# xuchang116/smCounter

Measured on NVIDIA B200. Metric: target_loci_called_per_sec, higher is better.
Workload: dtype int32+f64

## Files before the change

### smcounter_b200/csrc/smc_api.cu

```cuda
#include <chrono>
#include <cmath>
#include <cstdio>
#include <cstdlib>
#include <new>
#include <mutex>
#include <string>
#include <vector>

#include <nvtx3/nvToolsExt.h>

#include "smc_common.cuh"
#include "smc_sort.cuh"
#include "smc_pileup.cuh"
#include "smc_stats.cuh"

namespace {

struct NvtxRange {
    explicit NvtxRange(const char* name) { nvtxRangePushA(name); }
    ~NvtxRange() { nvtxRangePop(); }
};

thread_local std::string g_create_error;
static std::mutex g_link_mu;
// ... 341 lines not shown
        return SMC_E_CUDA;
    }
    if (device < 0 || device >= ndev) { g_create_error = "smc_ctx_create: bad device index"; return SMC_E_ARG; }
    smc_ctx* ctx = new (std::nothrow) smc_ctx();
    if (!ctx) { g_create_error = "smc_ctx_create: out of host memory"; return SMC_E_ARG; }
    ctx->device = device; ctx->prm = *params;
    if (const char* ev = getenv("SMC_CHUNK")) { long v = atol(ev); if (v >= 64 && v <= 1000000) ctx->chunk = (uint32_t)v; }
    auto fail = [&](const char* what, cudaError_t ce) {
        g_create_error = std::string(what) + ": " + cudaGetErrorString(ce);
        delete ctx; return SMC_E_CUDA;
    };
    if ((e = cudaSetDevice(device)) != cudaSuccess) return fail("cudaSetDevice", e);
    if ((e = cudaStreamCreateWithFlags(&ctx->st, cudaStreamNonBlocking)) != cudaSuccess) return fail("cudaStreamCreate", e);
    for (DevBuf* b : all_bufs(ctx)) b->st = ctx->st;
    {
        cudaMemPool_t pool;
        unsigned long long keep = ~0ull;
        if ((e = cudaDeviceGetDefaultMemPool(&pool, device)) != cudaSuccess) return fail("cudaDeviceGetDefaultMemPool", e);
        if ((e = cudaMemPoolSetAttribute(pool, cudaMemPoolAttrReleaseThreshold, &keep)) != cudaSuccess) return fail("cudaMemPoolSetAttribute", e);
    }
    for (auto& ev : ctx->ev) if ((e = cudaEventCreate(&ev)) != cudaSuccess) return fail("cudaEventCreate", e);
    if ((e = cudaStreamCreateWithFlags(&ctx->st_copy, cudaStreamNonBlocking)) != cudaSuccess) return fail("cudaStreamCreate", e);
    if ((e = cudaEventCreateWithFlags(&ctx->ev_scal, cudaEventDisableTiming)) != cudaSuccess) return fail("cudaEventCreate", e);
    if ((e = cudaEventCreateWithFlags(&ctx->ev_link, cudaEventDisableTiming)) != cudaSuccess) return fail("cudaEventCreate", e);
    if ((e = cudaEventCreateWithFlags(&ctx->ev_tmp, cudaEventDisableTiming)) != cudaSuccess) return fail("cudaEventCreate", e);
    if ((e = cudaEventCreateWithFlags(&ctx->ev_tmp2, cudaEventDisableTiming)) != cudaSuccess) return fail("cudaEventCreate", e);
    for (auto& ev : ctx->ev_chunk) if ((e = cudaEventCreateWithFlags(&ev, cudaEventDisableTiming)) != cudaSuccess) return fail("cudaEventCreate", e);
    std::vector<double> bq(256);
    for (int q = 0; q < 256; ++q) bq[q] = std::pow(10.0, -(double)q / 10.0);
    const size_t per = (size_t)(PCR_NMAX + 1) * (PCR_NMAX + 2) / 2;
    std::vector<double> pcr(3 * per);
    for (int k = 4; k <= 6; ++k)
        for (int n = 0; n <= PCR_NMAX; ++n)
            for (int c = 0; c <= n; ++c) {
                double ratio = ((double)c + 0.5) / ((double)n + 0.5 * (double)k);
                pcr[(size_t)(k - 4) * per + (size_t)n * (n + 1) / 2 + c] = std::pow(10.0, -6.0 * ratio);
            }
    if ((e = ctx->d_bqtab.ensure(256 * 8)) != cudaSuccess) return fail("cudaMalloc", e);
    if ((e = ctx->d_pcrtab.ensure(pcr.size() * 8)) != cudaSuccess) return fail("cudaMalloc", e);
    cudaMemcpy(ctx->d_bqtab.p, bq.data(), 256 * 8, cudaMemcpyHostToDevice);
    cudaMemcpy(ctx->d_pcrtab.p, pcr.data(), pcr.size() * 8, cudaMemcpyHostToDevice);
    if ((e = cudaFuncSetAttribute(k_merge_t<false>, cudaFuncAttributeMaxDynamicSharedMemorySize, KB_SMEM_BYTES)) != cudaSuccess)
        return fail("cudaFuncSetAttribute(k_merge)", e);
    if ((e = cudaFuncSetAttribute(k_merge_t<true>, cudaFuncAttributeMaxDynamicSharedMemorySize, KB_SMEM_BYTES)) != cudaSuccess)
        return fail("cudaFuncSetAttribute(k_merge list)", e);
    if ((e = cudaFuncSetAttribute(k_gather_t<false>, cudaFuncAttributeMaxDynamicSharedMemorySize, KA_SMEM_BYTES(false))) != cudaSuccess)
        return fail("cudaFuncSetAttribute(k_gather)", e);
    if ((e = cudaFuncSetAttribute(k_gather_t<true>, cudaFuncAttributeMaxDynamicSharedMemorySize, KA_SMEM_BYTES(true))) != cudaSuccess)
        return fail("cudaFuncSetAttribute(k_gather list)", e);
    cudaFuncSetAttribute(k_gather_t<false>, cudaFuncAttributePreferredSharedMemoryCarveout, cudaSharedmemCarveoutMaxShared);
    cudaFuncSetAttribute(k_gather_t<true>, cudaFuncAttributePreferredSharedMemoryCarveout, cudaSharedmemCarveoutMaxShared);
    cudaFuncSetAttribute(k_merge_t<false>, cudaFuncAttributePreferredSharedMemoryCarveout, cudaSharedmemCarveoutMaxShared);
    cudaFuncSetAttribute(k_merge_t<true>, cudaFuncAttributePreferredSharedMemoryCarveout, cudaSharedmemCarveoutMaxShared);
    if ((e = radix_sort_init()) != cudaSuccess) return fail("cudaFuncSetAttribute(k_radix_scatter)", e);
    if ((e = ctx->d_small.ensure(4096)) != cudaSuccess) return fail("cudaMalloc", e);
    *out = ctx;
    return SMC_OK;
}

extern "C" void smc_ctx_destroy(smc_ctx* ctx) {
    if (!ctx) return;
    cudaSetDevice(ctx->device);
    if (ctx->st_copy) cudaStreamSynchronize(ctx->st_copy);
    cudaStreamSynchronize(ctx->st);
    for (DevBuf* b : all_bufs(ctx)) b->release();
    cudaStreamSynchronize(ctx->st);
    for (auto& ev : ctx->ev) if (ev) cudaEventDestroy(ev);
    for (auto& ev : ctx->ev_chunk) if (ev) cudaEventDestroy(ev);
    if (ctx->ev_scal) cudaEventDestroy(ctx->ev_scal);
    if (ctx->ev_tmp) cudaEventDestroy(ctx->ev_tmp);
    if (ctx->ev_tmp2) cudaEventDestroy(ctx->ev_tmp2);
    if (ctx->ev_link) {
        std::lock_guard<std::mutex> lk(g_link_mu);
        if (ctx->device >= 0 && ctx->device < 64 && g_link_owner[ctx->device] == ctx) { g_link_owner[ctx->device] = nullptr; g_link_tail[ctx->device] = nullptr; }
        cudaEventDestroy(ctx->ev_link);
    }
    if (ctx->st_copy) cudaStreamDestroy(ctx->st_copy);
    if (ctx->st) cudaStreamDestroy(ctx->st);
    delete ctx;
}

static int pipe_chunks_for(const smc_reads_soa* R) {
    if (const char* ev = getenv("SMC_PIPE_CHUNKS")) { long v = atol(ev); if (v >= 1 && v <= SMC_PIPE_MAX) return (int)v; }
    const int64_t payload = R->seq_bytes + R->qual_bytes;
    if (R->n_reads < 65536 || payload < (96ll << 20)) return 1;
    const int64_t g = payload / (48ll << 20);
    return (int)(g < 2 ? 2 : g > 12 ? 12 : g);
}

static int upload_impl(smc_ctx* ctx, const smc_reads_soa* R, const smc_loci* Lc, const smc_umi_keep* K, bool pipelined) {
    if (!ctx) return SMC_E_ARG;
    NvtxRange nvtx_r("smc:upload");
    if (!R || !Lc) { ctx->err = "smc_upload: null reads/loci"; return SMC_E_ARG; }
    if (R->n_reads < 0 || Lc->n_loci < 0) { ctx->err = "smc_upload: negative size"; return SMC_E_ARG; }
    if (Lc->n_loci > SMC_MAX_LOCI) { ctx->err = "smc_upload: more than 4194302 loci in one batch"; return SMC_E_LIMIT; }
    if (R->n_reads > (1ll << 30) || R->seq_bytes >= (1ll << 32) || R->qual_bytes >= (1ll << 32) || R->n_cigar_words >= (1ll << 32)) {
        ctx->err = "smc_upload: batch exceeds 2^30 reads or 4 GiB of bases/qualities/cigar; split the batch"; return SMC_E_LIMIT;
    }
    CK(cudaSetDevice(ctx->device));
    ctx->uploaded = false; ctx->ran = false;
    const int64_t n = R->n_reads, nl = Lc->n_loci;
    const int G = pipelined ? pipe_chunks_for(R) : 1;
    ctx->pipe_n = 0;
    const bool split = pipelined && G > 1;
    cudaStream_t up_st = split ? ctx->st_copy : ctx->st;
    static const bool link_turns = [] { const char* ev = getenv("SMC_LINK_TURNS"); return !(ev && atoi(ev) == 0); }();
    std::unique_lock<std::mutex> link_lock(g_link_mu, std::defer_lock);
// ... 182 lines not shown
            LAUNCH(k_chunk_reads, 1, 32, 0, ctx->d_qual_poff.as<uint32_t>(), n, (uint32_t)R->qual_bytes, ctx->pipe_qual_chunk, G,
                   ctx->d_small.as<uint32_t>() + SW_CHUNK_READS);
        if (sbits == 2)
            LAUNCH(k_chunk_reads, 1, 32, 0, ctx->d_seq_poff.as<uint32_t>(), n, (uint32_t)R->seq_bytes, ctx->pipe_seq_chunk, G,
                   ctx->d_small.as<uint32_t>() + SW_CHUNK_READS_SEQ);
        grew = true;
        ALLOC_SYNC();
        for (int c = 0; c < G; ++c) {
            const int64_t s0 = std::min<int64_t>(R->seq_bytes, (int64_t)c * ctx->pipe_seq_chunk), s1 = std::min<int64_t>(R->seq_bytes, (int64_t)(c + 1) * ctx->pipe_seq_chunk);
            const int64_t q0 = std::min<int64_t>(R->qual_bytes, (int64_t)c * ctx->pipe_qual_chunk), q1 = std::min<int64_t>(R->qual_bytes, (int64_t)(c + 1) * ctx->pipe_qual_chunk);
            if (s1 > s0) CK(cudaMemcpyAsync(seq_up.as<uint8_t>() + s0, R->seq + s0, (size_t)(s1 - s0), cudaMemcpyHostToDevice, ctx->st_copy));
            if (q1 > q0) CK(cudaMemcpyAsync(qual_up.as<uint8_t>() + q0, R->qual + q0, (size_t)(q1 - q0), cudaMemcpyHostToDevice, ctx->st_copy));
            CK(cudaEventRecord(ctx->ev_chunk[c], ctx->st_copy));
            bytes += (s1 - s0) + (q1 - q0);
        }
        CK(cudaEventRecord(ctx->ev[1], ctx->st_copy));
        if (link_lock.owns_lock()) {
            CK(cudaEventRecord(ctx->ev_link, ctx->st_copy));
            g_link_tail[dv] = ctx->ev_link; g_link_owner[dv] = ctx;
        }
        ctx->pipe_n = G;
    }
#undef UP
#undef SYNC_UP
#undef ENSURE
#undef ALLOC_SYNC
    ctx->tm.pipe_chunks = pipelined ? G : 0;
    ctx->tm.bytes_h2d = bytes;
    ctx->uploaded = true;
    return SMC_OK;
}

extern "C" int smc_upload(smc_ctx* ctx, const smc_reads_soa* R, const smc_loci* Lc, const smc_umi_keep* K) {
    return upload_impl(ctx, R, Lc, K, false);
}

static int run_pileup_and_stats(smc_ctx* ctx, uint32_t n_tiles, int64_t NE);

extern "C" int smc_run_resident(smc_ctx* ctx) {
    if (!ctx) return SMC_E_ARG;
    if (!ctx->uploaded) { ctx->err = "smc_run_resident: nothing uploaded"; return SMC_E_STATE; }
    CK(cudaSetDevice(ctx->device));
    g_launches = 0;
    NvtxRange nvtx_r("smc:read_sort+prep+tile_events");
    const int64_t n = ctx->n_reads, nl = ctx->n_loci;
    const uint32_t n_tiles = (uint32_t)((nl + 31) / 32);
    uint32_t* small = ctx->d_small.as<uint32_t>();
    CK(cudaEventRecord(ctx->ev[2], ctx->st));
    int64_t NE = 0;
    int frag_bits_used = 32;
    if (n > 0 && nl > 0) {
        CK(ctx->d_k0.ensure((size_t)n * 8)); CK(ctx->d_k1.ensure((size_t)n * 8));
        CK(ctx->d_v0.ensure((size_t)n * 4)); CK(ctx->d_v1.ensure((size_t)n * 4));
        CK(ctx->d_hist.ensure(radix_hist_words(n) * 4 + 1024));
        CK(ctx->d_scan.ensure((size_t)std::max<int64_t>(radix_scan_words(n), scan_scratch_words(n + 1)) * 4 + 1024));
        uint64_t* k0 = ctx->d_k0.as<uint64_t>(); uint64_t* k1 = ctx->d_k1.as<uint64_t>();
        uint32_t* v0 = ctx->d_v0.as<uint32_t>(); uint32_t* v1 = ctx->d_v1.as<uint32_t>();
        int slot_bits = 4;
        while ((double)(1ll << slot_bits) < 1.1 * (double)n) ++slot_bits;
        int frag_bits = 1;
        while ((1ll << frag_bits) < n) ++frag_bits;
        frag_bits_used = frag_bits;
        CK(ctx->d_umi_table.ensure(((size_t)1 << slot_bits) * 8));
        CK(cudaMemsetAsync(ctx->d_umi_table.p, 0xff, ((size_t)1 << slot_bits) * 8, ctx->st));
        CK(cudaMemsetAsync(small + SW_FRAG_OR, 0, 8, ctx->st));
        LAUNCH(k_umi_slots, nblk(n, 256), 256, 0, ctx->d_umi.as<uint64_t>(), ctx->d_frag.as<uint32_t>(), n,
               ctx->d_umi_table.as<unsigned long long>(), (uint32_t)((1u << slot_bits) - 1u), frag_bits, k0, v0, (unsigned long long*)(small + SW_FRAG_OR));
        CK(cudaEventRecord(ctx->ev[11], ctx->st));
        if (radix_sort_bits(k0, v0, k1, v1, n, 0, slot_bits + frag_bits, ctx->d_hist.as<uint32_t>(), ctx->d_scan.as<uint32_t>(), ctx->st)) {
            std::swap(k0, k1); std::swap(v0, v1);
        }
        CK(cudaEventRecord(ctx->ev[12], ctx->st));
        ctx->tm.read_sort_passes = (slot_bits + frag_bits + RS_MAX_BITS - 1) / RS_MAX_BITS;
        const uint32_t* perm = v0;
        CK(ctx->d_urank.ensure((size_t)n * 4)); CK(ctx->d_frank.ensure((size_t)n * 4));
        CK(ctx->d_umi_of_urank.ensure((size_t)n * 8));
        uint32_t* uex = ctx->d_urank.as<uint32_t>(); uint32_t* fex = ctx->d_frank.as<uint32_t>();
        {
            const int64_t nbt = (n + SCAN_TILE - 1) / SCAN_TILE;
            uint32_t* scr = ctx->d_scan.as<uint32_t>();
            CK(cudaMemsetAsync(scr, 0, (size_t)(2 * nbt + 8) * 4, ctx->st));
            LAUNCH(k_rank_scan, (unsigned)nbt, SCAN_THREADS, 0, k0, frag_bits, n, ctx->d_umi.as<uint64_t>(), perm, uex, fex,
                   ctx->d_umi_of_urank.as<uint64_t>(), v1, reinterpret_cast<unsigned long long*>(scr + 2), scr, small + SW_N_UMI);
        }
        CK(ctx->d_recs.ensure((size_t)n * sizeof(ReadRec))); CK(ctx->d_grec.ensure((size_t)n * sizeof(GRec)));
        CK(cudaMemsetAsync(small + SW_N_TILE_EVENTS, 0, 32, ctx->st));
        PrepArgs P{};
        ctx->inv_ptr = v1;
        P.n_reads = n; P.inv = v1; P.urank = uex; P.frank = fex;
        P.ref_id = ctx->d_ref_id.as<int32_t>(); P.pos = ctx->d_pos.as<int32_t>(); P.flag = ctx->d_flag.as<uint16_t>();
        P.mapq = ctx->d_mapq.as<uint8_t>(); P.nm = ctx->d_nm.as<int32_t>(); P.l_seq = ctx->d_lseq.as<int32_t>();
        P.seq_off = ctx->d_seq_off.as<int64_t>(); P.qual_off = ctx->d_qual_off.as<int64_t>(); P.cigar_off = ctx->d_cig_off.as<int64_t>();
        P.n_cigar = ctx->d_ncig.as<uint16_t>(); P.cigar = ctx->d_cigar.as<uint32_t>();
        if (ctx->has_store) { P.store_lo = ctx->d_store_lo.as<int32_t>(); P.store_len = ctx->d_store_len.as<int32_t>(); }
        P.loci_key = ctx->d_loci_key.as<uint64_t>(); P.n_loci = nl;
        P.minMQ = ctx->prm.minMQ; P.primerDist = ctx->prm.primerDist; P.mismatchThr = ctx->prm.mismatchThr;
        P.recs = ctx->d_recs.as<ReadRec>(); P.grec = ctx->d_grec.as<GRec>(); P.gflags = small + SW_GFLAGS;
        if (ctx->pipe_n > 1) {
            CK(ctx->d_pipe_need.ensure((size_t)n));
            P.pipe_need = ctx->d_pipe_need.as<uint8_t>(); P.pipe_n = (uint32_t)ctx->pipe_n;
            P.pipe_seq_chunk = ctx->pipe_seq_chunk; P.pipe_qual_chunk = ctx->pipe_qual_chunk;
            if (ctx->qual_bits != 8) { P.qual_poff = ctx->d_qual_poff.as<uint32_t>(); P.qual_bits = ctx->qual_bits; }
            if (ctx->seq_bits == 2) P.seq_poff = ctx->d_seq_poff.as<uint32_t>();
        }
        CK(cudaEventRecord(ctx->ev[13], ctx->st));
        LAUNCH(k_read_prep, nblk(n, 256), 256, 0, P);
        CK(cudaEventRecord(ctx->ev[14], ctx->st));
        ctx->tm.read_prep_bytes = n * (int64_t)(4 + 4 + 2 + 1 + 4 + 4 + 8 + 8 + 8 + 2 + (ctx->has_store ? 8 : 0) + 4 + sizeof(ReadRec) + sizeof(GRec)) + 4 * ctx->n_cigar_words;
        if (ctx->ne_cap < 4 * n + 4096) ctx->ne_cap = 4 * n + 4096;
        for (int attempt = 0; attempt < 2; ++attempt) {
            if (ctx->ne_cap > 0xfffffff0ll) ctx->ne_cap = 0xfffffff0ll;
            CK(ctx->d_ek0.ensure((size_t)ctx->ne_cap * 8)); CK(ctx->d_ev0.ensure((size_t)ctx->ne_cap * 4));
            const int64_t nbt = (n + SCAN_TILE - 1) / SCAN_TILE;
            uint32_t* scr = ctx->d_scan.as<uint32_t>();
            CK(cudaMemsetAsync(scr, 0, (size_t)(2 * nbt + 8) * 4, ctx->st));
            LAUNCH(k_expand_scan, (unsigned)nbt, SCAN_THREADS, 0, ctx->d_recs.as<ReadRec>(), n, ctx->d_ek0.as<uint64_t>(), ctx->d_ev0.as<uint32_t>(),
                   (uint32_t)ctx->ne_cap, reinterpret_cast<unsigned long long*>(scr + 2), scr, small + SW_N_TILE_EVENTS);
            if (attempt == 1) break;
        uint32_t h[2], tot[5];
        unsigned long long frag_or = 0;
        CK(cudaMemcpyAsync(&frag_or, small + SW_FRAG_OR, 8, cudaMemcpyDeviceToHost, ctx->st));
        CK(cudaMemcpyAsync(h, small + SW_N_TILE_EVENTS, 8, cudaMemcpyDeviceToHost, ctx->st));
        CK(cudaMemcpyAsync(tot, small + SW_PACK_TOTALS, 20, cudaMemcpyDeviceToHost, ctx->st));
        CK(cudaStreamSynchronize(ctx->st));
        if (h[1] & GF_BAD_READ) { ctx->err = "a read has l_seq or clip length > 65535 (unsupported)"; return SMC_E_LIMIT; }
        if (h[1] & GF_BAD_STORE) {
            ctx->err = "stored window: store_lo must be even and >= 0, store_lo + store_len <= l_seq, reads with indels / clips inside must be "
                       "stored whole, and every target base of a read must lie inside its window";
            return SMC_E_ARG;
        }
        if (frag_or >> frag_bits_used) { ctx->err = "frag_id must be a dense id (< n_reads), numbered by first appearance"; return SMC_E_ARG; }
        if ((ctx->packed_seq && (int64_t)tot[ctx->seq_bits == 2 ? 4 : 0] != ctx->seq_bytes) || (ctx->packed_qual && (int64_t)tot[ctx->qual_bits != 8 ? 3 : 1] != ctx->qual_bytes) ||
            (ctx->packed_cigar && (int64_t)tot[2] != ctx->n_cigar_words)) {
            ctx->err = "packed payload (NULL offsets): seq_bytes / qual_bytes / n_cigar_words do not match the sums of (len+1)/2, len, n_cigar (len = store_len or l_seq)";
            return SMC_E_ARG;
        }
            NE = h[0];
            if (NE <= ctx->ne_cap) break;
            ctx->ne_cap = NE + NE / 8 + 4096;
        }
    }
    CK(cudaEventRecord(ctx->ev[3], ctx->st));
    CK(cudaEventRecord(ctx->ev[15], ctx->st));
    const uint64_t* ev_key_sorted = nullptr; const uint32_t* ev_read_sorted = nullptr;
    CK(ctx->d_tile_off.ensure((size_t)(n_tiles + 2) * 4)); CK(ctx->d_unit_cnt.ensure((size_t)(n_tiles + 2) * 4));
    CK(ctx->d_unit_off.ensure((size_t)(n_tiles + 2) * 4));
    if (NE > 0) {
        CK(ctx->d_ek1.ensure((size_t)NE * 8)); CK(ctx->d_ev1.ensure((size_t)NE * 4));
        CK(ctx->d_hist.ensure(radix_hist_words(NE) * 4 + 1024));
        CK(ctx->d_scan.ensure((size_t)std::max<int64_t>(radix_scan_words(NE), scan_scratch_words((int64_t)n_tiles + 2)) * 4 + 1024));
        int tile_bits = 0;
        while (((uint64_t)(n_tiles - 1) >> tile_bits) != 0) ++tile_bits;
        int res = radix_sort_bits(ctx->d_ek0.as<uint64_t>(), ctx->d_ev0.as<uint32_t>(), ctx->d_ek1.as<uint64_t>(), ctx->d_ev1.as<uint32_t>(),
                                  NE, 0, tile_bits, ctx->d_hist.as<uint32_t>(), ctx->d_scan.as<uint32_t>(), ctx->st);
        ev_key_sorted = res ? ctx->d_ek1.as<uint64_t>() : ctx->d_ek0.as<uint64_t>();
        ev_read_sorted = res ? ctx->d_ev1.as<uint32_t>() : ctx->d_ev0.as<uint32_t>();
    } else {
        CK(ctx->d_scan.ensure((size_t)scan_scratch_words((int64_t)n_tiles + 2) * 4 + 1024));
    }
    CK(cudaEventRecord(ctx->ev[16], ctx->st));
    LAUNCH(k_tile_offsets, nblk((int64_t)n_tiles + 1, 256), 256, 0, ev_key_sorted, NE, n_tiles, ctx->chunk, ctx->d_tile_off.as<uint32_t>(),
           ctx->d_unit_cnt.as<uint32_t>());
    exclusive_scan_u32(ctx->d_unit_cnt.as<uint32_t>(), ctx->d_unit_off.as<uint32_t>(), (int64_t)n_tiles + 1, ctx->d_scan.as<uint32_t>(),
                       nullptr, ctx->st);
    {
        const int64_t max_units = (int64_t)n_tiles + NE / ctx->chunk + 1;
        ctx->n_units_cap = (uint32_t)max_units;
        CK(ctx->d_unit_eb.ensure((size_t)max_units * 4)); CK(ctx->d_unit_ee.ensure((size_t)max_units * 4));
        CK(ctx->d_unit_tile.ensure((size_t)max_units * 4)); CK(ctx->d_unit_nfrag.ensure((size_t)max_units * 4));
        LAUNCH(k_unit_bounds, nblk(max_units, 256), 256, 0, ctx->d_tile_off.as<uint32_t>(), ctx->d_unit_off.as<uint32_t>(), n_tiles, ctx->chunk,
               ev_read_sorted, ctx->d_urank.as<uint32_t>(), ctx->d_unit_eb.as<uint32_t>(), ctx->d_unit_ee.as<uint32_t>(), ctx->d_unit_tile.as<uint32_t>(),
               ctx->n_units_cap);
    }
    ctx->tm.n_tile_events = NE;
    ctx->ev_read_sorted = ev_read_sorted;
    ctx->n_tiles = n_tiles; ctx->n_tile_events = NE;
    (void)ev_key_sorted;
    if (ctx->pipe_n > 1 && NE > 0) {
        const int G = ctx->pipe_n;
        uint32_t init[SMC_PIPE_MAX];
        for (int c = 0; c < SMC_PIPE_MAX; ++c) init[c] = ctx->n_units_cap;
        uint32_t* pd = small + SW_PIPE_BLOCKED;
        CK(cudaMemcpyAsync(pd, init, sizeof(init), cudaMemcpyHostToDevice, ctx->st));
        LAUNCH(k_pipe_unit_need, nblk((int64_t)ctx->n_units_cap * 32, 256), 256, 0, ctx->d_unit_eb.as<uint32_t>(),
               ctx->d_unit_ee.as<uint32_t>(), ev_read_sorted, ctx->d_pipe_need.as<uint8_t>(), ctx->n_units_cap, pd);
        uint32_t h[SMC_PIPE_MAX];
        CK(cudaMemcpyAsync(h, pd, sizeof(h), cudaMemcpyDeviceToHost, ctx->st));
        CK(cudaStreamSynchronize(ctx->st));
        uint32_t run = ctx->n_units_cap;
        for (int c = G - 1; c >= 0; --c) {
            if (c < G - 1) run = std::min(run, h[c]);
            ctx->pipe_end[c] = run;
        }
    }
    CK(cudaEventRecord(ctx->ev[4], ctx->st));
    return run_pileup_and_stats(ctx, n_tiles, NE);
}


static DynTab make_dyntab(smc_ctx* ctx) {
    uint32_t* small = ctx->d_small.as<uint32_t>();
    DynTab T;
    T.dkey = ctx->d_dkey.as<unsigned long long>(); T.dmask = ctx->dyn_cap - 1; T.drep_read = ctx->d_drep_read.as<uint32_t>();
    T.drep_qpos = ctx->d_drep_qpos.as<int32_t>(); T.dlen = ctx->d_dlen.as<int32_t>(); T.dcnt = ctx->d_dcnt.as<int32_t>();
    T.dlimb = ctx->d_dlimb.as<unsigned long long>(); T.diskey = ctx->d_diskey.as<uint8_t>(); T.dcount = small + SW_DYN_COUNT; T.gflags = small + SW_GFLAGS;
    T.seq = ctx->d_seq.as<uint8_t>(); T.seq_off = ctx->d_seq_off.as<int64_t>();
    T.spill = ctx->d_spill.as<SpillRec>(); T.spill_cap = ctx->spill_cap; T.spill_count = small + SW_SPILL_COUNT;
// ... 418 lines not shown
```

### smcounter_b200/csrc/smc_sort.cuh

```cuda
#pragma once
#include "smc_common.cuh"

#define SCAN_THREADS 256
#define SCAN_ITEMS   8
#define SCAN_TILE    (SCAN_THREADS * SCAN_ITEMS)

__global__ void __launch_bounds__(SCAN_THREADS)
k_scan_tile(const uint32_t* in, uint32_t* out, int64_t n, uint32_t* sums) {
    __shared__ uint32_t warp_tot[SCAN_THREADS / 32];
    int64_t base = (int64_t)blockIdx.x * SCAN_TILE + (int64_t)threadIdx.x * SCAN_ITEMS;
    uint32_t v[SCAN_ITEMS];
    uint32_t tsum = 0;
#pragma unroll
    for (int i = 0; i < SCAN_ITEMS; ++i) {
        v[i] = (base + i < n) ? in[base + i] : 0u;
        tsum += v[i];
    }
    uint32_t incl = tsum;
#pragma unroll
    for (int d = 1; d < 32; d <<= 1) {
        uint32_t t = __shfl_up_sync(FULL_MASK, incl, d);
        if (lane_id() >= (uint32_t)d) incl += t;
    }
    int w = threadIdx.x >> 5;
// ... 63 lines not shown
    for (int d = 1; d < 32; d <<= 1) {
        uint32_t t = __shfl_up_sync(FULL_MASK, incl, d);
        if (lane_id() >= (uint32_t)d) incl += t;
    }
    const int w = threadIdx.x >> 5;
    if (lane_id() == 31) warp_tot[w] = incl;
    __syncthreads();
    uint32_t woff = 0, blk = 0;
#pragma unroll
    for (int i = 0; i < SCAN_THREADS / 32; ++i) {
        uint32_t t = warp_tot[i];
        if (i < w) woff += t;
        blk += t;
    }
    if (threadIdx.x < 32) {
        const uint32_t prefix = (uint32_t)lb_resolve(desc, tile, blk);
        if (threadIdx.x == 0) {
            s_prefix = prefix;
            if (total && tile == gridDim.x - 1) *total = prefix + blk;
        }
    }
    __syncthreads();
    uint32_t run = s_prefix + woff + incl - tsum;
#pragma unroll
    for (int i = 0; i < SCAN_ITEMS; ++i) {
        if (base + i < n) out[base + i] = run;
        run += v[i];
    }
}

static inline int64_t scan_scratch_words(int64_t n) {
    return 2 * ((n + SCAN_TILE - 1) / SCAN_TILE) + 8;
}

static thread_local int g_launches = 0;

static void exclusive_scan_u32(const uint32_t* in, uint32_t* out, int64_t n, uint32_t* scratch, uint32_t* total,
                               cudaStream_t st) {
    if (n <= 0) {
        if (total) cudaMemsetAsync(total, 0, sizeof(uint32_t), st);
        return;
    }
    const int64_t nb = (n + SCAN_TILE - 1) / SCAN_TILE;
    if (nb == 1) {
        k_scan_tile<<<1, SCAN_THREADS, 0, st>>>(in, out, n, total);
        ++g_launches;
        return;
    }
    cudaMemsetAsync(scratch, 0, (size_t)(2 * nb + 8) * 4, st);
    k_scan_lb<<<(unsigned)nb, SCAN_THREADS, 0, st>>>(in, out, n, reinterpret_cast<unsigned long long*>(scratch + 2), scratch, total);
    ++g_launches;
}

#define RS_WARPS   8
#define RS_THREADS (RS_WARPS * 32)
#define RS_ITEMS   8
#define RS_TILE    (RS_THREADS * RS_ITEMS)
#define RS_MAX_BITS 11

__device__ __forceinline__ int64_t rs_index(int64_t tile_base, int w, int it, int lane) {
    return tile_base + (int64_t)w * (32 * RS_ITEMS) + it * 32 + lane;
}

template <int BITS>
__global__ void __launch_bounds__(RS_THREADS)
k_radix_hist(const uint64_t* __restrict__ keys, int64_t n, int shift, uint32_t* __restrict__ hist, uint32_t nblocks) {
    constexpr uint32_t ND = 1u << BITS;
    __shared__ uint32_t h[ND];
    for (uint32_t d = threadIdx.x; d < ND; d += RS_THREADS) h[d] = 0;
    __syncthreads();
    int w = threadIdx.x >> 5, lane = threadIdx.x & 31;
    int64_t tb = (int64_t)blockIdx.x * RS_TILE;
#pragma unroll
    for (int it = 0; it < RS_ITEMS; ++it) {
        int64_t i = rs_index(tb, w, it, lane);
        if (i < n) atomicAdd(&h[(uint32_t)(keys[i] >> shift) & (ND - 1u)], 1u);
    }
    __syncthreads();
    for (uint32_t d = threadIdx.x; d < ND; d += RS_THREADS) hist[(size_t)d * nblocks + blockIdx.x] = h[d];
}

template <int BITS>
__global__ void __launch_bounds__(RS_THREADS)
k_radix_scatter(const uint64_t* __restrict__ keys, const uint32_t* __restrict__ vals, uint64_t* __restrict__ keys_out,
                uint32_t* __restrict__ vals_out, int64_t n, int shift, const uint32_t* __restrict__ hist_scanned,
                uint32_t nblocks) {
    constexpr uint32_t ND = 1u << BITS;
    extern __shared__ uint32_t wh_s[];
    int w = threadIdx.x >> 5, lane = threadIdx.x & 31;
    for (uint32_t i = threadIdx.x; i < RS_WARPS * ND; i += RS_THREADS) wh_s[i] = 0;
    __syncthreads();
    uint32_t* wh = wh_s + (size_t)w * ND;
    int64_t tb = (int64_t)blockIdx.x * RS_TILE;
    uint64_t k[RS_ITEMS];
    uint32_t v[RS_ITEMS];
#pragma unroll
    for (int it = 0; it < RS_ITEMS; ++it) {
        int64_t i = rs_index(tb, w, it, lane);
        if (i < n) {
            k[it] = keys[i];
            v[it] = vals[i];
            atomicAdd(&wh[(uint32_t)(k[it] >> shift) & (ND - 1u)], 1u);
        }
    }
    __syncthreads();
    for (uint32_t d = threadIdx.x; d < ND; d += RS_THREADS) {
        uint32_t run = hist_scanned[(size_t)d * nblocks + blockIdx.x];
#pragma unroll
        for (int ww = 0; ww < RS_WARPS; ++ww) {
            uint32_t t = wh_s[(size_t)ww * ND + d];
            wh_s[(size_t)ww * ND + d] = run;
            run += t;
        }
    }
    __syncthreads();
    uint32_t lt = (1u << lane) - 1u;
#pragma unroll
    for (int it = 0; it < RS_ITEMS; ++it) {
        int64_t i = rs_index(tb, w, it, lane);
        bool valid = i < n;
        uint32_t active = __ballot_sync(FULL_MASK, valid);
        if (valid) {
            uint32_t d = (uint32_t)(k[it] >> shift) & (ND - 1u);
            uint32_t peers = __match_any_sync(active, d);
            uint32_t rank = __popc(peers & lt);
            int leader = __ffs(peers) - 1;
            uint32_t off = 0;
            if (lane == leader) {
                off = wh[d];
                wh[d] = off + __popc(peers);
            }
            off = __shfl_sync(peers, off, leader);
            keys_out[off + rank] = k[it];
            vals_out[off + rank] = v[it];
        }
        __syncwarp();
    }
}

static inline size_t radix_hist_words(int64_t n) { return ((size_t)1 << RS_MAX_BITS) * (size_t)((n + RS_TILE - 1) / RS_TILE) + 256; }
static inline int64_t radix_scan_words(int64_t n) { return scan_scratch_words((int64_t)radix_hist_words(n)); }

template <int BITS>
static void radix_pass(const uint64_t* ki, const uint32_t* vi, uint64_t* ko, uint32_t* vo, int64_t n, int shift, uint32_t* hist,
                       uint32_t* scan_scratch, cudaStream_t st) {
    const uint32_t nblocks = (uint32_t)((n + RS_TILE - 1) / RS_TILE);
    constexpr size_t smem = (size_t)RS_WARPS * (1u << BITS) * 4;
    k_radix_hist<BITS><<<nblocks, RS_THREADS, 0, st>>>(ki, n, shift, hist, nblocks);
    ++g_launches;
    exclusive_scan_u32(hist, hist, (int64_t)(1u << BITS) * nblocks, scan_scratch, nullptr, st);
    k_radix_scatter<BITS><<<nblocks, RS_THREADS, smem, st>>>(ki, vi, ko, vo, n, shift, hist, nblocks);
    ++g_launches;
}

static cudaError_t radix_sort_init() {
    return cudaFuncSetAttribute(k_radix_scatter<RS_MAX_BITS>, cudaFuncAttributeMaxDynamicSharedMemorySize, RS_WARPS * (1 << RS_MAX_BITS) * 4);
}

static int radix_sort_bits(uint64_t* k0, uint32_t* v0, uint64_t* k1, uint32_t* v1, int64_t n, int lo_bit, int nbits, uint32_t* hist,
                           uint32_t* scan_scratch, cudaStream_t st) {
    if (n <= 1 || nbits <= 0) return 0;
    const int npass = (nbits + RS_MAX_BITS - 1) / RS_MAX_BITS;
    int width = (nbits + npass - 1) / npass;
    if (width < 8) width = 8;
    int cur = 0;
    for (int done = 0; done < nbits; done += width) {
        uint64_t* ki = cur ? k1 : k0; uint32_t* vi = cur ? v1 : v0;
        uint64_t* ko = cur ? k0 : k1; uint32_t* vo = cur ? v0 : v1;
        const int shift = lo_bit + done;
        switch (width) {
            case 8:  radix_pass<8>(ki, vi, ko, vo, n, shift, hist, scan_scratch, st); break;
            case 9:  radix_pass<9>(ki, vi, ko, vo, n, shift, hist, scan_scratch, st); break;
            case 10: radix_pass<10>(ki, vi, ko, vo, n, shift, hist, scan_scratch, st); break;
            default: radix_pass<11>(ki, vi, ko, vo, n, shift, hist, scan_scratch, st); break;
        }
        cur ^= 1;
    }
    return cur;
}

__global__ void k_or_and_u32(const uint32_t* __restrict__ a, int64_t n, unsigned long long* __restrict__ out) {
    unsigned long long o = 0;
    for (int64_t i = (int64_t)blockIdx.x * blockDim.x + threadIdx.x; i < n; i += (int64_t)gridDim.x * blockDim.x) o |= a[i];
#pragma unroll
    for (int s = 16; s > 0; s >>= 1) o |= __shfl_xor_sync(FULL_MASK, o, s);
    if (lane_id() == 0 && o) atomicOr(&out[0], o);
}
```

Measured before the change: 3.630 million.

## Replace per-pass histogram/scan/scatter radix sort with onesweep decoupled-lookback sort

Replaces the three-kernel-per-pass LSD radix sort (histogram, global scan, scatter) with a single upsweep kernel that builds histograms for all passes at once, followed by one onesweep kernel per pass. Each onesweep tile takes a dynamic tile id, ranks its keys in shared memory, gets its global offsets through decoupled lookback on per-digit descriptors, and writes out locally sorted runs so the global stores are coalesced. The aim is fewer launches and fewer passes over the keys per sort. In exchange, tiles spin-wait on their predecessors, the scratch space grows with tiles times digits, and the maximum digit width drops to 9 bits, which may add passes for wide keys.

```diff
diff --git a/smcounter_b200/csrc/smc_api.cu b/smcounter_b200/csrc/smc_api.cu
--- a/smcounter_b200/csrc/smc_api.cu
+++ b/smcounter_b200/csrc/smc_api.cu
@@ -417,7 +417,7 @@
     cudaFuncSetAttribute(k_gather_t<true>, cudaFuncAttributePreferredSharedMemoryCarveout, cudaSharedmemCarveoutMaxShared);
     cudaFuncSetAttribute(k_merge_t<false>, cudaFuncAttributePreferredSharedMemoryCarveout, cudaSharedmemCarveoutMaxShared);
     cudaFuncSetAttribute(k_merge_t<true>, cudaFuncAttributePreferredSharedMemoryCarveout, cudaSharedmemCarveoutMaxShared);
-    if ((e = radix_sort_init()) != cudaSuccess) return fail("cudaFuncSetAttribute(k_radix_scatter)", e);
+    if ((e = radix_sort_init()) != cudaSuccess) return fail("cudaFuncSetAttribute(k_onesweep)", e);
     if ((e = ctx->d_small.ensure(4096)) != cudaSuccess) return fail("cudaMalloc", e);
     *out = ctx;
     return SMC_OK;
@@ -706,8 +706,7 @@
     if (n > 0 && nl > 0) {
         CK(ctx->d_k0.ensure((size_t)n * 8)); CK(ctx->d_k1.ensure((size_t)n * 8));
         CK(ctx->d_v0.ensure((size_t)n * 4)); CK(ctx->d_v1.ensure((size_t)n * 4));
-        CK(ctx->d_hist.ensure(radix_hist_words(n) * 4 + 1024));
-        CK(ctx->d_scan.ensure((size_t)std::max<int64_t>(radix_scan_words(n), scan_scratch_words(n + 1)) * 4 + 1024));
+        CK(ctx->d_scan.ensure((size_t)scan_scratch_words(n + 1) * 4 + 1024));
         uint64_t* k0 = ctx->d_k0.as<uint64_t>(); uint64_t* k1 = ctx->d_k1.as<uint64_t>();
         uint32_t* v0 = ctx->d_v0.as<uint32_t>(); uint32_t* v1 = ctx->d_v1.as<uint32_t>();
         int slot_bits = 4;
@@ -715,17 +714,18 @@
         int frag_bits = 1;
         while ((1ll << frag_bits) < n) ++frag_bits;
         frag_bits_used = frag_bits;
+        CK(ctx->d_hist.ensure(radix_scratch_words(n, slot_bits + frag_bits) * 4));
         CK(ctx->d_umi_table.ensure(((size_t)1 << slot_bits) * 8));
         CK(cudaMemsetAsync(ctx->d_umi_table.p, 0xff, ((size_t)1 << slot_bits) * 8, ctx->st));
         CK(cudaMemsetAsync(small + SW_FRAG_OR, 0, 8, ctx->st));
         LAUNCH(k_umi_slots, nblk(n, 256), 256, 0, ctx->d_umi.as<uint64_t>(), ctx->d_frag.as<uint32_t>(), n,
                ctx->d_umi_table.as<unsigned long long>(), (uint32_t)((1u << slot_bits) - 1u), frag_bits, k0, v0, (unsigned long long*)(small + SW_FRAG_OR));
         CK(cudaEventRecord(ctx->ev[11], ctx->st));
-        if (radix_sort_bits(k0, v0, k1, v1, n, 0, slot_bits + frag_bits, ctx->d_hist.as<uint32_t>(), ctx->d_scan.as<uint32_t>(), ctx->st)) {
+        if (radix_sort_bits(k0, v0, k1, v1, n, 0, slot_bits + frag_bits, ctx->d_hist.as<uint32_t>(), ctx->st)) {
             std::swap(k0, k1); std::swap(v0, v1);
         }
         CK(cudaEventRecord(ctx->ev[12], ctx->st));
-        ctx->tm.read_sort_passes = (slot_bits + frag_bits + RS_MAX_BITS - 1) / RS_MAX_BITS;
+        ctx->tm.read_sort_passes = rs_plan(slot_bits + frag_bits).npass;
         const uint32_t* perm = v0;
         CK(ctx->d_urank.ensure((size_t)n * 4)); CK(ctx->d_frank.ensure((size_t)n * 4));
         CK(ctx->d_umi_of_urank.ensure((size_t)n * 8));
@@ -801,12 +801,12 @@
     CK(ctx->d_unit_off.ensure((size_t)(n_tiles + 2) * 4));
     if (NE > 0) {
         CK(ctx->d_ek1.ensure((size_t)NE * 8)); CK(ctx->d_ev1.ensure((size_t)NE * 4));
-        CK(ctx->d_hist.ensure(radix_hist_words(NE) * 4 + 1024));
-        CK(ctx->d_scan.ensure((size_t)std::max<int64_t>(radix_scan_words(NE), scan_scratch_words((int64_t)n_tiles + 2)) * 4 + 1024));
+        CK(ctx->d_scan.ensure((size_t)scan_scratch_words((int64_t)n_tiles + 2) * 4 + 1024));
         int tile_bits = 0;
         while (((uint64_t)(n_tiles - 1) >> tile_bits) != 0) ++tile_bits;
+        CK(ctx->d_hist.ensure(radix_scratch_words(NE, tile_bits) * 4));
         int res = radix_sort_bits(ctx->d_ek0.as<uint64_t>(), ctx->d_ev0.as<uint32_t>(), ctx->d_ek1.as<uint64_t>(), ctx->d_ev1.as<uint32_t>(),
-                                  NE, 0, tile_bits, ctx->d_hist.as<uint32_t>(), ctx->d_scan.as<uint32_t>(), ctx->st);
+                                  NE, 0, tile_bits, ctx->d_hist.as<uint32_t>(), ctx->st);
         ev_key_sorted = res ? ctx->d_ek1.as<uint64_t>() : ctx->d_ek0.as<uint64_t>();
         ev_read_sorted = res ? ctx->d_ev1.as<uint32_t>() : ctx->d_ev0.as<uint32_t>();
     } else {
diff --git a/smcounter_b200/csrc/smc_sort.cuh b/smcounter_b200/csrc/smc_sort.cuh
--- a/smcounter_b200/csrc/smc_sort.cuh
+++ b/smcounter_b200/csrc/smc_sort.cuh
@@ -139,131 +139,229 @@
     ++g_launches;
 }
 
-#define RS_WARPS   8
-#define RS_THREADS (RS_WARPS * 32)
-#define RS_ITEMS   8
-#define RS_TILE    (RS_THREADS * RS_ITEMS)
-#define RS_MAX_BITS 11
-
-__device__ __forceinline__ int64_t rs_index(int64_t tile_base, int w, int it, int lane) {
-    return tile_base + (int64_t)w * (32 * RS_ITEMS) + it * 32 + lane;
+#define RS_MAX_BITS 9
+#define RS_WARPS    8
+#define RS_THREADS  (RS_WARPS * 32)
+#define RS_ITEMS    16
+#define RS_TILE     (RS_THREADS * RS_ITEMS)
+#define RS_UP_TILE  (4 * RS_TILE)
+#define RS_CTRL     64
+
+struct RsPlan { int npass, bits; };
+static inline RsPlan rs_plan(int nbits) {
+    const int npass = (nbits + RS_MAX_BITS - 1) / RS_MAX_BITS;
+    const int widest = (nbits + npass - 1) / npass;
+    return {npass, widest < 8 ? 8 : widest};
+}
+__host__ __device__ __forceinline__ int rs_pass_shift(int lo_bit, int nbits, int npass, int p) {
+    return lo_bit + p * (nbits / npass) + (p < nbits % npass ? p : nbits % npass);
+}
+__host__ __device__ __forceinline__ int rs_pass_width(int nbits, int npass, int p) { return nbits / npass + (p < nbits % npass); }
+
+__device__ __forceinline__ uint32_t rs_block_excl(uint32_t x, uint32_t* wsum) {
+    const int w = threadIdx.x >> 5;
+    uint32_t incl = x;
+#pragma unroll
+    for (int d = 1; d < 32; d <<= 1) {
+        const uint32_t t = __shfl_up_sync(FULL_MASK, incl, d);
+        if (lane_id() >= (uint32_t)d) incl += t;
+    }
+    if (lane_id() == 31) wsum[w] = incl;
+    __syncthreads();
+    uint32_t off = 0;
+#pragma unroll
+    for (int i = 0; i < RS_WARPS; ++i) off += i < w ? wsum[i] : 0u;
+    __syncthreads();
+    return off + incl - x;
 }
 
 template <int BITS>
 __global__ void __launch_bounds__(RS_THREADS)
-k_radix_hist(const uint64_t* __restrict__ keys, int64_t n, int shift, uint32_t* __restrict__ hist, uint32_t nblocks) {
+k_radix_upsweep(const uint64_t* __restrict__ keys, int64_t n, int lo_bit, int nbits, int npass, uint32_t* hist, uint32_t* done) {
     constexpr uint32_t ND = 1u << BITS;
-    __shared__ uint32_t h[ND];
-    for (uint32_t d = threadIdx.x; d < ND; d += RS_THREADS) h[d] = 0;
-    __syncthreads();
-    int w = threadIdx.x >> 5, lane = threadIdx.x & 31;
-    int64_t tb = (int64_t)blockIdx.x * RS_TILE;
-#pragma unroll
-    for (int it = 0; it < RS_ITEMS; ++it) {
-        int64_t i = rs_index(tb, w, it, lane);
-        if (i < n) atomicAdd(&h[(uint32_t)(keys[i] >> shift) & (ND - 1u)], 1u);
-    }
-    __syncthreads();
-    for (uint32_t d = threadIdx.x; d < ND; d += RS_THREADS) hist[(size_t)d * nblocks + blockIdx.x] = h[d];
+    extern __shared__ uint32_t h[];
+    __shared__ uint32_t wsum[RS_WARPS];
+    __shared__ bool s_last;
+    for (uint32_t i = threadIdx.x; i < (uint32_t)npass * ND; i += RS_THREADS) h[i] = 0;
+    __syncthreads();
+    for (int64_t b = (int64_t)blockIdx.x * RS_UP_TILE; b < min(n, ((int64_t)blockIdx.x + 1) * RS_UP_TILE); b += RS_TILE) {
+        uint64_t k[RS_ITEMS];
+#pragma unroll
+        for (int it = 0; it < RS_ITEMS; ++it) {
+            const int64_t i = b + it * RS_THREADS + threadIdx.x;
+            k[it] = i < n ? keys[i] : 0;
+        }
+        for (int p = 0; p < npass; ++p) {
+            const int sh = rs_pass_shift(lo_bit, nbits, npass, p);
+            const uint32_t m = (1u << rs_pass_width(nbits, npass, p)) - 1u;
+#pragma unroll
+            for (int it = 0; it < RS_ITEMS; ++it)
+                if (b + it * RS_THREADS + threadIdx.x < n) atomicAdd(&h[p * ND + ((uint32_t)(k[it] >> sh) & m)], 1u);
+        }
+    }
+    __syncthreads();
+    for (uint32_t i = threadIdx.x; i < (uint32_t)npass * ND; i += RS_THREADS)
+        if (h[i]) atomicAdd(&hist[i], h[i]);
+    __threadfence();
+    __syncthreads();
+    if (threadIdx.x == 0) s_last = atomicAdd(done, 1u) == gridDim.x - 1;
+    __syncthreads();
+    if (!s_last) return;
+    __threadfence();
+    constexpr int DPT = ND / RS_THREADS;
+    for (int p = 0; p < npass; ++p) {
+        uint32_t* hp = hist + (size_t)p * ND + threadIdx.x * DPT;
+        uint32_t c[DPT], sum = 0;
+#pragma unroll
+        for (int j = 0; j < DPT; ++j) { c[j] = __ldcg(hp + j); sum += c[j]; }
+        uint32_t run = rs_block_excl(sum, wsum);
+#pragma unroll
+        for (int j = 0; j < DPT; ++j) { hp[j] = run; run += c[j]; }
+    }
 }
 
 template <int BITS>
 __global__ void __launch_bounds__(RS_THREADS)
-k_radix_scatter(const uint64_t* __restrict__ keys, const uint32_t* __restrict__ vals, uint64_t* __restrict__ keys_out,
-                uint32_t* __restrict__ vals_out, int64_t n, int shift, const uint32_t* __restrict__ hist_scanned,
-                uint32_t nblocks) {
+k_onesweep(const uint64_t* __restrict__ keys, const uint32_t* __restrict__ vals, uint64_t* __restrict__ keys_out,
+           uint32_t* __restrict__ vals_out, int64_t n, int shift, uint32_t mask, const uint32_t* __restrict__ digit_base,
+           unsigned long long* desc, uint32_t* tile_counter) {
     constexpr uint32_t ND = 1u << BITS;
-    extern __shared__ uint32_t wh_s[];
-    int w = threadIdx.x >> 5, lane = threadIdx.x & 31;
-    for (uint32_t i = threadIdx.x; i < RS_WARPS * ND; i += RS_THREADS) wh_s[i] = 0;
-    __syncthreads();
-    uint32_t* wh = wh_s + (size_t)w * ND;
-    int64_t tb = (int64_t)blockIdx.x * RS_TILE;
+    constexpr int DPT = ND / RS_THREADS;
+    extern __shared__ __align__(16) unsigned char rs_smem[];
+    uint64_t* s_key = reinterpret_cast<uint64_t*>(rs_smem);
+    uint32_t* s_val = reinterpret_cast<uint32_t*>(s_key + RS_TILE);
+    uint32_t* s_wh = s_val + RS_TILE;
+    uint32_t* s_off = s_wh + RS_WARPS * ND;
+    __shared__ uint32_t wsum[RS_WARPS];
+    __shared__ uint32_t s_tile;
+    if (threadIdx.x == 0) s_tile = atomicAdd(tile_counter, 1u);
+    for (uint32_t i = threadIdx.x; i < RS_WARPS * ND; i += RS_THREADS) s_wh[i] = 0;
+    __syncthreads();
+    const uint32_t tile = s_tile;
+    const int w = threadIdx.x >> 5, lane = threadIdx.x & 31;
+    const int64_t tb = (int64_t)tile * RS_TILE;
+    const int tile_n = (int)min((int64_t)RS_TILE, n - tb);
     uint64_t k[RS_ITEMS];
-    uint32_t v[RS_ITEMS];
+    uint32_t v[RS_ITEMS], r[RS_ITEMS];
+    uint32_t* wh = s_wh + w * ND;
+    const uint32_t lt = (1u << lane) - 1u;
 #pragma unroll
     for (int it = 0; it < RS_ITEMS; ++it) {
-        int64_t i = rs_index(tb, w, it, lane);
-        if (i < n) {
-            k[it] = keys[i];
-            v[it] = vals[i];
-            atomicAdd(&wh[(uint32_t)(k[it] >> shift) & (ND - 1u)], 1u);
-        }
-    }
-    __syncthreads();
-    for (uint32_t d = threadIdx.x; d < ND; d += RS_THREADS) {
-        uint32_t run = hist_scanned[(size_t)d * nblocks + blockIdx.x];
-#pragma unroll
-        for (int ww = 0; ww < RS_WARPS; ++ww) {
-            uint32_t t = wh_s[(size_t)ww * ND + d];
-            wh_s[(size_t)ww * ND + d] = run;
-            run += t;
-        }
-    }
-    __syncthreads();
-    uint32_t lt = (1u << lane) - 1u;
+        const int i = w * (32 * RS_ITEMS) + it * 32 + lane;
+        if (i < tile_n) { k[it] = keys[tb + i]; v[it] = vals[tb + i]; }
+    }
 #pragma unroll
     for (int it = 0; it < RS_ITEMS; ++it) {
-        int64_t i = rs_index(tb, w, it, lane);
-        bool valid = i < n;
-        uint32_t active = __ballot_sync(FULL_MASK, valid);
+        const bool valid = w * (32 * RS_ITEMS) + it * 32 + lane < tile_n;
+        const uint32_t active = __ballot_sync(FULL_MASK, valid);
         if (valid) {
-            uint32_t d = (uint32_t)(k[it] >> shift) & (ND - 1u);
-            uint32_t peers = __match_any_sync(active, d);
-            uint32_t rank = __popc(peers & lt);
-            int leader = __ffs(peers) - 1;
-            uint32_t off = 0;
-            if (lane == leader) {
-                off = wh[d];
-                wh[d] = off + __popc(peers);
+            const uint32_t d = (uint32_t)(k[it] >> shift) & mask;
+            const uint32_t peers = __match_any_sync(active, d);
+            const int leader = __ffs(peers) - 1;
+            uint32_t base = 0;
+            if (lane == leader) { base = wh[d]; wh[d] = base + __popc(peers); }
+            r[it] = __shfl_sync(peers, base, leader) + __popc(peers & lt);
+        }
+        __syncwarp();
+    }
+    __syncthreads();
+    uint32_t cnt[DPT], sum = 0;
+#pragma unroll
+    for (int j = 0; j < DPT; ++j) {
+        const uint32_t d = threadIdx.x * DPT + j;
+        uint32_t run = 0;
+#pragma unroll
+        for (int ww = 0; ww < RS_WARPS; ++ww) { const uint32_t t = s_wh[ww * ND + d]; s_wh[ww * ND + d] = run; run += t; }
+        cnt[j] = run;
+        sum += run;
+    }
+    unsigned long long* my = desc + (size_t)tile * ND + threadIdx.x * DPT;
+#pragma unroll
+    for (int j = 0; j < DPT; ++j)
+        *reinterpret_cast<volatile unsigned long long*>(my + j) = (tile ? LB_AGG : LB_INCL) | cnt[j];
+    uint32_t start = rs_block_excl(sum, wsum);
+#pragma unroll
+    for (int j = 0; j < DPT; ++j) {
+        const uint32_t d = threadIdx.x * DPT + j;
+#pragma unroll
+        for (int ww = 0; ww < RS_WARPS; ++ww) s_wh[ww * ND + d] += start;
+        unsigned long long prefix = 0;
+        if (tile) {
+            for (int64_t t = (int64_t)tile - 1;; --t) {
+                unsigned long long dv;
+                do { dv = *reinterpret_cast<volatile unsigned long long*>(desc + (size_t)t * ND + d); } while ((dv >> 62) == 0ull);
+                prefix += dv & LB_VAL;
+                if ((dv >> 62) == 2ull) break;
             }
-            off = __shfl_sync(peers, off, leader);
-            keys_out[off + rank] = k[it];
-            vals_out[off + rank] = v[it];
-        }
-        __syncwarp();
-    }
-}
-
-static inline size_t radix_hist_words(int64_t n) { return ((size_t)1 << RS_MAX_BITS) * (size_t)((n + RS_TILE - 1) / RS_TILE) + 256; }
-static inline int64_t radix_scan_words(int64_t n) { return scan_scratch_words((int64_t)radix_hist_words(n)); }
+            *reinterpret_cast<volatile unsigned long long*>(my + j) = LB_INCL | (prefix + cnt[j]);
+        }
+        s_off[d] = digit_base[d] + (uint32_t)prefix - start;
+        start += cnt[j];
+    }
+    __syncthreads();
+#pragma unroll
+    for (int it = 0; it < RS_ITEMS; ++it) {
+        const int i = w * (32 * RS_ITEMS) + it * 32 + lane;
+        if (i < tile_n) {
+            const uint32_t pos = s_wh[w * ND + ((uint32_t)(k[it] >> shift) & mask)] + r[it];
+            s_key[pos] = k[it];
+            s_val[pos] = v[it];
+        }
+    }
+    __syncthreads();
+    for (int i = threadIdx.x; i < tile_n; i += RS_THREADS) {
+        const uint64_t key = s_key[i];
+        const uint32_t o = s_off[(uint32_t)(key >> shift) & mask] + (uint32_t)i;
+        keys_out[o] = key;
+        vals_out[o] = s_val[i];
+    }
+}
 
 template <int BITS>
-static void radix_pass(const uint64_t* ki, const uint32_t* vi, uint64_t* ko, uint32_t* vo, int64_t n, int shift, uint32_t* hist,
-                       uint32_t* scan_scratch, cudaStream_t st) {
-    const uint32_t nblocks = (uint32_t)((n + RS_TILE - 1) / RS_TILE);
-    constexpr size_t smem = (size_t)RS_WARPS * (1u << BITS) * 4;
-    k_radix_hist<BITS><<<nblocks, RS_THREADS, 0, st>>>(ki, n, shift, hist, nblocks);
+static constexpr size_t rs_onesweep_smem() { return (size_t)RS_TILE * 12 + ((size_t)RS_WARPS + 1) * (1u << BITS) * 4; }
+
+static inline size_t radix_scratch_words(int64_t n, int nbits) {
+    if (n <= 1 || nbits <= 0) return RS_CTRL;
+    const RsPlan pl = rs_plan(nbits);
+    const size_t nd = (size_t)1 << pl.bits, tiles = (size_t)((n + RS_TILE - 1) / RS_TILE);
+    return RS_CTRL + (size_t)pl.npass * nd + 2 * (size_t)pl.npass * tiles * nd;
+}
+
+static cudaError_t radix_sort_init() {
+    cudaError_t e = cudaFuncSetAttribute(k_onesweep<8>, cudaFuncAttributeMaxDynamicSharedMemorySize, (int)rs_onesweep_smem<8>());
+    if (e == cudaSuccess) e = cudaFuncSetAttribute(k_onesweep<RS_MAX_BITS>, cudaFuncAttributeMaxDynamicSharedMemorySize, (int)rs_onesweep_smem<RS_MAX_BITS>());
+    return e;
+}
+
+template <int BITS>
+static void radix_sort_run(const RsPlan& pl, uint64_t* k0, uint32_t* v0, uint64_t* k1, uint32_t* v1, int64_t n, int lo_bit, int nbits,
+                           uint32_t* scratch, cudaStream_t st) {
+    constexpr size_t nd = (size_t)1 << BITS;
+    const uint32_t tiles = (uint32_t)((n + RS_TILE - 1) / RS_TILE);
+    uint32_t* hist = scratch + RS_CTRL;
+    unsigned long long* desc = reinterpret_cast<unsigned long long*>(hist + (size_t)pl.npass * nd);
+    cudaMemsetAsync(scratch, 0, radix_scratch_words(n, nbits) * 4, st);
+    k_radix_upsweep<BITS><<<(unsigned)((n + RS_UP_TILE - 1) / RS_UP_TILE), RS_THREADS, (size_t)pl.npass * nd * 4, st>>>(
+        k0, n, lo_bit, nbits, pl.npass, hist, scratch);
     ++g_launches;
-    exclusive_scan_u32(hist, hist, (int64_t)(1u << BITS) * nblocks, scan_scratch, nullptr, st);
-    k_radix_scatter<BITS><<<nblocks, RS_THREADS, smem, st>>>(ki, vi, ko, vo, n, shift, hist, nblocks);
-    ++g_launches;
-}
-
-static cudaError_t radix_sort_init() {
-    return cudaFuncSetAttribute(k_radix_scatter<RS_MAX_BITS>, cudaFuncAttributeMaxDynamicSharedMemorySize, RS_WARPS * (1 << RS_MAX_BITS) * 4);
-}
-
-static int radix_sort_bits(uint64_t* k0, uint32_t* v0, uint64_t* k1, uint32_t* v1, int64_t n, int lo_bit, int nbits, uint32_t* hist,
-                           uint32_t* scan_scratch, cudaStream_t st) {
+    for (int p = 0; p < pl.npass; ++p) {
+        const bool odd = p & 1;
+        k_onesweep<BITS><<<tiles, RS_THREADS, rs_onesweep_smem<BITS>(), st>>>(
+            odd ? k1 : k0, odd ? v1 : v0, odd ? k0 : k1, odd ? v0 : v1, n, rs_pass_shift(lo_bit, nbits, pl.npass, p),
+            (1u << rs_pass_width(nbits, pl.npass, p)) - 1u, hist + (size_t)p * nd, desc + (size_t)p * tiles * nd, scratch + 1 + p);
+        ++g_launches;
+    }
+}
+
+static int radix_sort_bits(uint64_t* k0, uint32_t* v0, uint64_t* k1, uint32_t* v1, int64_t n, int lo_bit, int nbits, uint32_t* scratch,
+                           cudaStream_t st) {
     if (n <= 1 || nbits <= 0) return 0;
-    const int npass = (nbits + RS_MAX_BITS - 1) / RS_MAX_BITS;
-    int width = (nbits + npass - 1) / npass;
-    if (width < 8) width = 8;
-    int cur = 0;
-    for (int done = 0; done < nbits; done += width) {
-        uint64_t* ki = cur ? k1 : k0; uint32_t* vi = cur ? v1 : v0;
-        uint64_t* ko = cur ? k0 : k1; uint32_t* vo = cur ? v0 : v1;
-        const int shift = lo_bit + done;
-        switch (width) {
-            case 8:  radix_pass<8>(ki, vi, ko, vo, n, shift, hist, scan_scratch, st); break;
-            case 9:  radix_pass<9>(ki, vi, ko, vo, n, shift, hist, scan_scratch, st); break;
-            case 10: radix_pass<10>(ki, vi, ko, vo, n, shift, hist, scan_scratch, st); break;
-            default: radix_pass<11>(ki, vi, ko, vo, n, shift, hist, scan_scratch, st); break;
-        }
-        cur ^= 1;
-    }
-    return cur;
+    const RsPlan pl = rs_plan(nbits);
+    switch (pl.bits) {
+        case 8:  radix_sort_run<8>(pl, k0, v0, k1, v1, n, lo_bit, nbits, scratch, st); break;
+        default: radix_sort_run<RS_MAX_BITS>(pl, k0, v0, k1, v1, n, lo_bit, nbits, scratch, st); break;
+    }
+    return pl.npass & 1;
 }
 
 __global__ void k_or_and_u32(const uint32_t* __restrict__ a, int64_t n, unsigned long long* __restrict__ out) {
```

Measured after the change: 3.708 million, median of 6. 2.2% higher.
